# nihalsid/retrieval-fuse

Measured on AMD Instinct MI355X. Metric: 64^3 TSDF chunks/sec (retrieve+attend+refine), higher is better.
Workload: dtype f32

## Files before the change

### retrieval-fuse_amd/csrc/attention_fused.hip

```cpp
#include "common.h"
#include "attn_row.h"
#include "split_operand.h"
#include "philox.h"


typedef __attribute__((address_space(1))) const void* rf_gptr;
typedef __attribute__((address_space(3))) void* rf_lptr;

#define AM_HID 128
#define AM_OUT 32
#define AM_WAVES 16
#define AM_BUF_FLOATS (AM_HID * AM_HID)

static __host__ __device__ inline size_t am_layer_off(int n_in, int layer) {
    size_t o = 0;
    if (layer > 0) o += (size_t)n_in * AM_HID;
    if (layer > 1) o += (size_t)AM_HID * AM_HID;
    if (layer > 2) o += (size_t)AM_HID * AM_HID;
    if (layer > 3) o += (size_t)AM_HID * AM_OUT;
    return o;
}
static __host__ __device__ inline size_t am_bias_off(int n_in, int layer) { return am_layer_off(n_in, 4) + (size_t)layer * AM_HID; }

extern "C" size_t rf_attn_mlp_packed_floats(int n_in) { return am_bias_off(n_in, 3) + AM_OUT; }

struct AmPackArgs {
    const float* w[4];
    const float* b[4];
    float* img;
    int n_in;
};

__global__ void k_attn_mlp_pack(AmPackArgs a) {
    const size_t total = am_bias_off(a.n_in, 3) + AM_OUT;
    for (size_t i = (size_t)blockIdx.x * blockDim.x + threadIdx.x; i < total; i += (size_t)gridDim.x * blockDim.x) {
        float v;
        if (i >= am_layer_off(a.n_in, 4)) {
            const size_t bi = i - am_layer_off(a.n_in, 4);
            const int layer = (int)(bi / AM_HID) > 3 ? 3 : (int)(bi / AM_HID);
            v = a.b[layer][bi - (size_t)layer * AM_HID];
        } else {
            int layer = 0;
            while (layer < 3 && i >= am_layer_off(a.n_in, layer + 1)) ++layer;
            const size_t li = i - am_layer_off(a.n_in, layer);
            const int nin = layer == 0 ? a.n_in : AM_HID;
            const int ibn = layer == 3 ? AM_OUT / 16 : AM_HID / 16;
            const int r = (int)(li & 3), lane = (int)((li >> 2) & 63);
            const int ib = (int)((li >> 8) % ibn), kb = (int)((li >> 8) / ibn);
            v = a.w[layer][(size_t)(ib * 16 + (lane & 15)) * nin + kb * 16 + 4 * (lane >> 4) + r];
        }
        a.img[i] = v;
    }
}

extern "C" int rf_attn_mlp_pack(const float* w1, const float* b1, const float* w2, const float* b2, const float* w3, const float* b3,
                                const float* w4, const float* b4, int n_in, float* packed, void* stream) {
    RF_REQUIRE(w1 && b1 && w2 && b2 && w3 && b3 && w4 && b4 && packed, RF_E_INVALID, "rf_attn_mlp_pack: null pointer");
    RF_REQUIRE(n_in >= 16 && n_in <= AM_HID && n_in % 16 == 0, RF_E_UNSUPPORTED, "rf_attn_mlp_pack: n_in %d must be a multiple of 16 in 16..128", n_in);
    AmPackArgs a;
    a.w[0] = w1; a.w[1] = w2; a.w[2] = w3; a.w[3] = w4;
    a.b[0] = b1; a.b[1] = b2; a.b[2] = b3; a.b[3] = b4;
    a.img = packed; a.n_in = n_in;
    return rf_launch<k_attn_mlp_pack>("rf_attn_mlp_pack", dim3(256), dim3(256), (hipStream_t)stream, a);
}

struct AmArgs {
    const float* src;
    const float* img;
    const float* img2;
    float* out;
    int mode;
    int nrows, n_in, ntiles;
    int kv, c, s, t;
};

template <int IB>
__device__ __forceinline__ void am_layer(const float* wbuf, int kbn, const f32x4 (&hin)[8], f32x4 (&acc)[8], int lane) {
    constexpr int GRP = 2;
    constexpr int NG = IB / GRP;
    const float4* wv = reinterpret_cast<const float4*>(wbuf) + lane;
#pragma unroll
    for (int ib = 0; ib < IB; ++ib) acc[ib] = (f32x4){0.f, 0.f, 0.f, 0.f};
    float4 aw[2][GRP];
#pragma unroll
    for (int i = 0; i < GRP; ++i) aw[0][i] = wv[i * 64];
#pragma unroll
    for (int kb = 0; kb < 8; ++kb) {
        if (kb < kbn) {
#pragma unroll
            for (int gi = 0; gi < NG; ++gi) {
                const int st = kb * NG + gi, cur = st & 1, nxt = cur ^ 1;
                if (st + 1 < 8 * NG) {
#pragma unroll
                    for (int i = 0; i < GRP; ++i) aw[nxt][i] = wv[((st + 1) * GRP + i) * 64];
                }
#pragma unroll
                for (int i = 0; i < GRP; ++i) acc[gi * GRP + i] = __builtin_amdgcn_mfma_f32_16x16x4f32(aw[cur][i].x, hin[kb][0], acc[gi * GRP + i], 0, 0, 0);
#pragma unroll
                for (int i = 0; i < GRP; ++i) acc[gi * GRP + i] = __builtin_amdgcn_mfma_f32_16x16x4f32(aw[cur][i].y, hin[kb][1], acc[gi * GRP + i], 0, 0, 0);
#pragma unroll
                for (int i = 0; i < GRP; ++i) acc[gi * GRP + i] = __builtin_amdgcn_mfma_f32_16x16x4f32(aw[cur][i].z, hin[kb][2], acc[gi * GRP + i], 0, 0, 0);
#pragma unroll
                for (int i = 0; i < GRP; ++i) acc[gi * GRP + i] = __builtin_amdgcn_mfma_f32_16x16x4f32(aw[cur][i].w, hin[kb][3], acc[gi * GRP + i], 0, 0, 0);
            }
        }
    }
}

__global__ __launch_bounds__(AM_WAVES * 64) void k_attn_mlp(AmArgs a) {
    extern __shared__ __attribute__((aligned(16))) float smem[];
    const int tid = threadIdx.x, lane = tid & 63;
    const int wave = __builtin_amdgcn_readfirstlane(tid >> 6);
    const int g = lane >> 4, j = lane & 15;
    const int kb0 = a.n_in >> 4;

    auto dma_layer = [&](int layer) {
        const int npiece = layer == 0 ? kb0 * 8 : (layer == 3 ? (AM_HID / 16) * (AM_OUT / 16) : 64);
        const float* src = a.img + am_layer_off(a.n_in, layer);
        float* dst = smem + (layer & 1) * AM_BUF_FLOATS;
        for (int q = wave; q < npiece; q += AM_WAVES)
            __builtin_amdgcn_global_load_lds((rf_gptr)(src + q * 256 + lane * 4), (rf_lptr)(dst + q * 256), 16, 0, 0);
    };
    const float4* bias4 = reinterpret_cast<const float4*>(a.img + am_layer_off(a.n_in, 4));

    dma_layer(0);
    const int nwt = (a.ntiles + AM_WAVES - 1) / AM_WAVES;
    for (int wt = blockIdx.x; wt < nwt; wt += gridDim.x) {
        const int rt = wt * AM_WAVES + wave;
        const bool live = rt < a.ntiles;
        int row = rt * 16 + j;
        if (row >= a.nrows) row = a.nrows - 1;
        if (row < 0) row = 0;
        size_t orow = (size_t)row;
        f32x4 hin[8];
        if (a.mode == 0) {
            const float* p = a.src + (size_t)row * a.n_in + 4 * g;
#pragma unroll
            for (int kb = 0; kb < 8; ++kb) {
                if (kb < kb0) {
                    const float4 v = *reinterpret_cast<const float4*>(p + kb * 16);
                    hin[kb] = (f32x4){v.x, v.y, v.z, v.w};
                } else {
                    hin[kb] = (f32x4){0.f, 0.f, 0.f, 0.f};
                }
            }
        } else {
            const int r = a.s >> 1, t = a.t, q = a.s / t;
            const int r3 = r * r * r;
            const int vol = row / r3, prow = row - vol * r3;
            const int p2 = prow % r, p1 = (prow / r) % r, p0 = prow / (r * r);
            const int bb = vol / a.kv, k = vol - bb * a.kv;
            orow = ((size_t)bb * r3 + prow) * a.kv + k;
            const int d0 = 2 * p0 + (g & 1), d1 = 2 * p1, d2 = 2 * p2;
            const size_t t3 = (size_t)t * t * t;
            const size_t patch = (((size_t)vol * q + d0 / t) * q + d1 / t) * q + d2 / t;
            const float* p = a.src + (patch * a.c + (g >> 1)) * t3 + ((size_t)(d0 % t) * t + (d1 % t)) * t + (d2 % t);
#pragma unroll
            for (int kb = 0; kb < 8; ++kb) {
                if (kb < kb0) {
                    const float2 lo = *reinterpret_cast<const float2*>(p + (size_t)(2 * kb) * t3);
                    const float2 hi = *reinterpret_cast<const float2*>(p + (size_t)(2 * kb) * t3 + t);
                    hin[kb] = (f32x4){lo.x, lo.y, hi.x, hi.y};
                } else {
                    hin[kb] = (f32x4){0.f, 0.f, 0.f, 0.f};
                }
            }
        }

        f32x4 acc[8];
#pragma unroll
        for (int layer = 0; layer < 4; ++layer) {
            __syncthreads();
            if (layer < 3) dma_layer(layer + 1);
            else if (wt + (int)gridDim.x < nwt) dma_layer(0);
            const float* wbuf = smem + (layer & 1) * AM_BUF_FLOATS;
            if (layer < 3) {
                am_layer<8>(wbuf, layer == 0 ? kb0 : 8, hin, acc, lane);
#pragma unroll
                for (int ib = 0; ib < 8; ++ib) {
                    const float4 bz = bias4[layer * 32 + ib * 4 + g];
                    f32x4 v = acc[ib];
                    v[0] += bz.x; v[1] += bz.y; v[2] += bz.z; v[3] += bz.w;
#pragma unroll
                    for (int e = 0; e < 4; ++e) v[e] = v[e] > 0.f ? v[e] : v[e] * 0.01f;
                    hin[ib] = v;
                }
            } else {
                am_layer<2>(wbuf, 8, hin, acc, lane);
                if (live && rt * 16 + j < a.nrows) {
#pragma unroll
                    for (int ib = 0; ib < 2; ++ib) {
                        const float4 bz = bias4[3 * 32 + ib * 4 + g];
                        const float4 o = make_float4(acc[ib][0] + bz.x, acc[ib][1] + bz.y, acc[ib][2] + bz.z, acc[ib][3] + bz.w);
                        *reinterpret_cast<float4*>(a.out + orow * AM_OUT + ib * 16 + 4 * g) = o;
                    }
                }
            }
        }
    }
}


static __host__ __device__ inline int ams_steps(int n_in, int layer) { return layer == 0 ? (n_in / 16 + 1) / 2 : 4; }
static __host__ __device__ inline int ams_ibn(int layer) { return layer == 3 ? AM_OUT / 16 : AM_HID / 16; }
static __host__ __device__ inline size_t ams_layer_off(int n_in, int layer) {
    size_t o = 0;
    for (int l = 0; l < layer; ++l) o += (size_t)ams_steps(n_in, l) * ams_ibn(l) * 2 * 256;
    return o;
}
extern "C" size_t rf_attn_mlp_split_packed_floats(int n_in) { return ams_layer_off(n_in, 4); }

struct AmsPackArgs {
    const float* w[4];
    float* img;
    int n_in;
};

__global__ void k_attn_mlp_split_pack(AmsPackArgs a) {
    const size_t total = ams_layer_off(a.n_in, 4) / 4;
    for (size_t i = (size_t)blockIdx.x * blockDim.x + threadIdx.x; i < total; i += (size_t)gridDim.x * blockDim.x) {
        int layer = 0;
        while (layer < 3 && i * 4 >= ams_layer_off(a.n_in, layer + 1)) ++layer;
        const size_t li = i - ams_layer_off(a.n_in, layer) / 4;
        const int nin = layer == 0 ? a.n_in : AM_HID, ibn = ams_ibn(layer);
        const int lane = (int)(li & 63), piece = (int)((li >> 6) & 1);
        const int ib = (int)((li >> 7) % ibn), t = (int)((li >> 7) / ibn);
        const int feat = ib * 16 + (lane & 15), g = lane >> 4;
        h8 out;
#pragma unroll
        for (int j = 0; j < 8; ++j) {
            const int k = 16 * (2 * t + (j >> 2)) + 4 * g + (j & 3);
            _Float16 h, l;
            rf_split_weight(k < nin ? (double)a.w[layer][(size_t)feat * nin + k] : 0.0, h, l);
            out[j] = piece == 0 ? h : l;
        }
        reinterpret_cast<h8*>(a.img)[i] = out;
    }
}

extern "C" int rf_attn_mlp_split_pack(const float* w1, const float* w2, const float* w3, const float* w4, int n_in, float* packed, void* stream) {
    RF_REQUIRE(w1 && w2 && w3 && w4 && packed, RF_E_INVALID, "rf_attn_mlp_split_pack: null pointer");
    RF_REQUIRE(n_in >= 16 && n_in <= AM_HID && n_in % 16 == 0, RF_E_UNSUPPORTED, "rf_attn_mlp_split_pack: n_in %d must be a multiple of 16 in 16..128", n_in);
    AmsPackArgs a;
    a.w[0] = w1; a.w[1] = w2; a.w[2] = w3; a.w[3] = w4; a.img = packed; a.n_in = n_in;
    return rf_launch<k_attn_mlp_split_pack>("rf_attn_mlp_split_pack", dim3(256), dim3(256), (hipStream_t)stream, a);
}

typedef float am_f2 __attribute__((ext_vector_type(2)));
__device__ __forceinline__ void ams_split4(const f32x4& v, h8& h, h8& l, int o) {
#pragma unroll
    for (int e = 0; e < 4; e += 2) {
        const am_f2 s2 = (am_f2){v[e], v[e + 1]} * (am_f2){SPLIT_ACT_SCALE, SPLIT_ACT_SCALE};
        am_f2 x;
        x.x = rf_clamp_f16(s2.x);
        x.y = rf_clamp_f16(s2.y);
        const am_f2 xl = x * (am_f2){SPLIT_LO, SPLIT_LO};
        const _Float16 ha = (_Float16)x.x, hb = (_Float16)x.y;
        h[o + e] = ha; h[o + e + 1] = hb;
        l[o + e] = (_Float16)fmaf(-SPLIT_LO, (float)ha, xl.x);
        l[o + e + 1] = (_Float16)fmaf(-SPLIT_LO, (float)hb, xl.y);
    }
}

template <int IB>
__device__ __forceinline__ void ams_layer(const float* wbuf, int tn, const h8 (&bh)[4], const h8 (&bl)[4], f32x4 (&hi)[8], f32x4 (&lo)[8], int lane) {
    const h8* wv = reinterpret_cast<const h8*>(wbuf) + lane;
#pragma unroll
    for (int ib = 0; ib < IB; ++ib) { hi[ib] = (f32x4){0.f, 0.f, 0.f, 0.f}; lo[ib] = (f32x4){0.f, 0.f, 0.f, 0.f}; }
    h8 wh[2], wl[2];
    wh[0] = wv[0]; wl[0] = wv[64];
#pragma unroll
    for (int t = 0; t < 4; ++t) {
        if (t < tn) {
#pragma unroll
            for (int ib = 0; ib < IB; ++ib) {
                const int st = t * IB + ib, cur = st & 1, nxt = cur ^ 1;
                if (st + 1 < 4 * IB) { wh[nxt] = wv[(st + 1) * 128]; wl[nxt] = wv[(st + 1) * 128 + 64]; }
                hi[ib] = __builtin_amdgcn_mfma_f32_16x16x32_f16(wh[cur], bh[t], hi[ib], 0, 0, 0);
                lo[ib] = __builtin_amdgcn_mfma_f32_16x16x32_f16(wh[cur], bl[t], lo[ib], 0, 0, 0);
                lo[ib] = __builtin_amdgcn_mfma_f32_16x16x32_f16(wl[cur], bh[t], lo[ib], 0, 0, 0);
            }
        }
    }
}

#define AMS_WAVES 12
__global__ __launch_bounds__(AMS_WAVES * 64) void k_attn_mlp_split(AmArgs a) {
    extern __shared__ __attribute__((aligned(16))) float smem[];
    const int tid = threadIdx.x, lane = tid & 63;
    const int wave = __builtin_amdgcn_readfirstlane(tid >> 6);
    const int g = lane >> 4, j = lane & 15;
    const int kb0 = a.n_in >> 4, t0n = (kb0 + 1) >> 1;

    auto dma_layer = [&](int layer) {
        const int npiece = ams_steps(a.n_in, layer) * ams_ibn(layer) * 2;
        const float* src = a.img2 + ams_layer_off(a.n_in, layer);
        float* dst = smem + (layer & 1) * AM_BUF_FLOATS;
        for (int q = wave; q < npiece; q += AMS_WAVES)
            __builtin_amdgcn_global_load_lds((rf_gptr)(src + q * 256 + lane * 4), (rf_lptr)(dst + q * 256), 16, 0, 0);
    };
    const float4* bias4 = reinterpret_cast<const float4*>(a.img + am_layer_off(a.n_in, 4));

    dma_layer(0);
    const int nwt = (a.ntiles + AMS_WAVES - 1) / AMS_WAVES;
    for (int wt = blockIdx.x; wt < nwt; wt += gridDim.x) {
        const int rt = wt * AMS_WAVES + wave;
        const bool live = rt < a.ntiles;
        int row = rt * 16 + j;
        if (row >= a.nrows) row = a.nrows - 1;
        if (row < 0) row = 0;
        size_t orow = (size_t)row;
        h8 bh[4], bl[4];
#pragma unroll
        for (int t = 0; t < 4; ++t) { bh[t] = (h8){0, 0, 0, 0, 0, 0, 0, 0}; bl[t] = bh[t]; }
        if (a.mode == 0) {
            const float* p = a.src + (size_t)row * a.n_in + 4 * g;
#pragma unroll
            for (int kb = 0; kb < 8; ++kb) {
                if (kb < kb0) {
                    const float4 v = *reinterpret_cast<const float4*>(p + kb * 16);
                    ams_split4((f32x4){v.x, v.y, v.z, v.w}, bh[kb >> 1], bl[kb >> 1], 4 * (kb & 1));
                }
            }
        } else {
            const int r = a.s >> 1, t = a.t, q = a.s / t;
            const int r3 = r * r * r;
            const int vol = row / r3, prow = row - vol * r3;
            const int p2 = prow % r, p1 = (prow / r) % r, p0 = prow / (r * r);
            const int bb = vol / a.kv, k = vol - bb * a.kv;
            orow = ((size_t)bb * r3 + prow) * a.kv + k;
            const int d0 = 2 * p0 + (g & 1), d1 = 2 * p1, d2 = 2 * p2;
            const size_t t3 = (size_t)t * t * t;
            const size_t patch = (((size_t)vol * q + d0 / t) * q + d1 / t) * q + d2 / t;
            const float* p = a.src + (patch * a.c + (g >> 1)) * t3 + ((size_t)(d0 % t) * t + (d1 % t)) * t + (d2 % t);
#pragma unroll
            for (int kb = 0; kb < 8; ++kb) {
                if (kb < kb0) {
                    const float2 lo2 = *reinterpret_cast<const float2*>(p + (size_t)(2 * kb) * t3);
                    const float2 hi2 = *reinterpret_cast<const float2*>(p + (size_t)(2 * kb) * t3 + t);
                    ams_split4((f32x4){lo2.x, lo2.y, hi2.x, hi2.y}, bh[kb >> 1], bl[kb >> 1], 4 * (kb & 1));
                }
            }
        }

        f32x4 hi[8], lo[8];
#pragma unroll
        for (int layer = 0; layer < 4; ++layer) {
            __syncthreads();
            if (layer < 3) dma_layer(layer + 1);
            else if (wt + (int)gridDim.x < nwt) dma_layer(0);
            const float* wbuf = smem + (layer & 1) * AM_BUF_FLOATS;
            if (layer < 3) {
                ams_layer<8>(wbuf, layer == 0 ? t0n : 4, bh, bl, hi, lo, lane);
#pragma unroll
                for (int ib = 0; ib < 8; ++ib) {
                    const float4 bz = bias4[layer * 32 + ib * 4 + g];
                    const am_f2 c2 = {1.0f / SPLIT_LO, 1.0f / SPLIT_LO}, s2 = {0.01f, 0.01f};
                    const am_f2 va = __builtin_elementwise_fma((am_f2){lo[ib][0], lo[ib][1]}, c2, (am_f2){hi[ib][0], hi[ib][1]}) + (am_f2){bz.x, bz.y};
                    const am_f2 vb = __builtin_elementwise_fma((am_f2){lo[ib][2], lo[ib][3]}, c2, (am_f2){hi[ib][2], hi[ib][3]}) + (am_f2){bz.z, bz.w};
                    const am_f2 na = va * s2, nb = vb * s2;
                    const f32x4 v = {rf_max(va.x, na.x), rf_max(va.y, na.y), rf_max(vb.x, nb.x), rf_max(vb.y, nb.y)};
                    ams_split4(v, bh[ib >> 1], bl[ib >> 1], 4 * (ib & 1));
                }
            } else {
                ams_layer<2>(wbuf, 4, bh, bl, hi, lo, lane);
                if (live && rt * 16 + j < a.nrows) {
#pragma unroll
                    for (int ib = 0; ib < 2; ++ib) {
                        const float4 bz = bias4[3 * 32 + ib * 4 + g];
                        const float4 o = make_float4(rf_split_join(hi[ib][0], lo[ib][0]) + bz.x, rf_split_join(hi[ib][1], lo[ib][1]) + bz.y,
                                                     rf_split_join(hi[ib][2], lo[ib][2]) + bz.z, rf_split_join(hi[ib][3], lo[ib][3]) + bz.w);
                        *reinterpret_cast<float4*>(a.out + orow * AM_OUT + ib * 16 + 4 * g) = o;
                    }
                }
            }
        }
    }
}

static int am_launch(const AmArgs& a, hipStream_t st) {
    constexpr size_t lds = 2 * AM_BUF_FLOATS * sizeof(float);
    if (a.img2) return rf_launch<k_attn_mlp_split>("rf_attn_mlp", dim3(rf_blocks(a.ntiles, AMS_WAVES, 256)), dim3(AMS_WAVES * 64), lds, lds, st, a);
    return rf_launch<k_attn_mlp>("rf_attn_mlp", dim3(rf_blocks(a.ntiles, AM_WAVES, 256)), dim3(AM_WAVES * 64), lds, lds, st, a);
}

static int am_rows(const float* x, int rows, int n_in, const float* packed, const float* packed_split, float* out, void* stream);
extern "C" int rf_attn_mlp_rows(const float* x, int rows, int n_in, const float* packed, float* out, void* stream) {
    return am_rows(x, rows, n_in, packed, nullptr, out, stream);
}
extern "C" int rf_attn_mlp_split_rows(const float* x, int rows, int n_in, const float* packed, const float* packed_split, float* out, void* stream) {
    RF_REQUIRE(packed_split, RF_E_INVALID, "rf_attn_mlp_split_rows: null split image");
    return am_rows(x, rows, n_in, packed, packed_split, out, stream);
}
static int am_rows(const float* x, int rows, int n_in, const float* packed, const float* packed_split, float* out, void* stream) {
    RF_REQUIRE(x && packed && out && rows > 0, RF_E_INVALID, "rf_attn_mlp_rows: bad arguments");
    RF_REQUIRE(n_in >= 16 && n_in <= AM_HID && n_in % 16 == 0, RF_E_UNSUPPORTED, "rf_attn_mlp_rows: n_in %d must be a multiple of 16 in 16..128", n_in);
    AmArgs a;
    a.src = x; a.img = packed; a.img2 = packed_split; a.out = out; a.mode = 0; a.nrows = rows; a.n_in = n_in; a.ntiles = (rows + 15) / 16;
    a.kv = 1; a.c = 0; a.s = 0; a.t = 0;
    return am_launch(a, (hipStream_t)stream);
}

static int am_volume(const float* src, int b, int kv, int c, int s, int t, const float* packed, const float* packed_split, float* out, void* stream);
extern "C" int rf_attn_mlp_volume(const float* src, int b, int kv, int c, int s, int t, const float* packed, float* out, void* stream) {
    return am_volume(src, b, kv, c, s, t, packed, nullptr, out, stream);
}
extern "C" int rf_attn_mlp_split_volume(const float* src, int b, int kv, int c, int s, int t, const float* packed, const float* packed_split, float* out, void* stream) {
    RF_REQUIRE(packed_split, RF_E_INVALID, "rf_attn_mlp_split_volume: null split image");
    return am_volume(src, b, kv, c, s, t, packed, packed_split, out, stream);
}
static int am_volume(const float* src, int b, int kv, int c, int s, int t, const float* packed, const float* packed_split, float* out, void* stream) {
    RF_REQUIRE(src && packed && out && b > 0 && kv > 0 && c > 0 && s > 0 && t > 0, RF_E_INVALID, "rf_attn_mlp_volume: bad arguments");
    RF_REQUIRE(s % 2 == 0 && t % 2 == 0 && s % t == 0, RF_E_INVALID, "rf_attn_mlp_volume: edges s=%d t=%d must be even and t | s", s, t);
    RF_REQUIRE(c % 2 == 0 && c * 8 <= AM_HID, RF_E_UNSUPPORTED, "rf_attn_mlp_volume: %d channels (need an even count <= 16)", c);
    const long long rows = (long long)b * kv * (s / 2) * (s / 2) * (s / 2);
    RF_REQUIRE(rows < (1ll << 31) - 16, RF_E_UNSUPPORTED, "rf_attn_mlp_volume: too many rows");
    AmArgs a;
    a.src = src; a.img = packed; a.img2 = packed_split; a.out = out; a.mode = 1; a.nrows = (int)rows; a.n_in = c * 8; a.ntiles = (int)((rows + 15) / 16);
    a.kv = kv; a.c = c; a.s = s; a.t = t;
    return am_launch(a, (hipStream_t)stream);
}

__device__ __forceinline__ void rf_gumbel_row(unsigned long long seed, unsigned long long offset, int row, int K, float (&g)[RF_MAX_K]) {
#pragma unroll
    for (int q = 0; q < RF_MAX_K / 4; ++q) {
        if (4 * q < K) {
            unsigned c[4] = {(unsigned)row, (unsigned)q, (unsigned)offset, (unsigned)(offset >> 32)};
            rf_philox4x32_10(c, (unsigned)seed, (unsigned)(seed >> 32));
#pragma unroll
            for (int j = 0; j < 4; ++j) {
                const float u = ((float)(c[j] >> 8) + 0.5f) * (1.0f / 16777216.0f);
                g[4 * q + j] = -logf(-logf(u));
            }
        }
    }
}

__global__ __launch_bounds__(256) void k_attn_weights(const float* __restrict__ xf, const float* __restrict__ pf, const float* __restrict__ noise,
                                                      unsigned long long* __restrict__ rng, int rows, int K, int f, int mode, float sharpness,
                                                      float* __restrict__ w_out, float* __restrict__ sw_out, float* __restrict__ scores_out,
                                                      float* __restrict__ noise_out) {
    const unsigned long long seed = rng ? rng[0] : 0ull, offset = rng ? rng[1] : 0ull;
    for (int row = blockIdx.x * blockDim.x + threadIdx.x; row < rows; row += gridDim.x * blockDim.x) {
        float sc[RF_MAX_K], w[RF_MAX_K], sw, g[RF_MAX_K];
        const float* nrow = noise ? noise + (size_t)row * K : nullptr;
        if (!noise && mode == RF_ATTN_GUMBEL_HARD) {
            rf_gumbel_row(seed, offset, row, K, g);
            nrow = g;
        }
        rf_attn_row_weights(xf + (size_t)row * f, pf + (size_t)row * K * f, nrow, K, f, mode, sharpness, sc, w, sw);
#pragma unroll
        for (int k = 0; k < RF_MAX_K; ++k) {
            if (k < K) {
                w_out[(size_t)row * K + k] = w[k];
                if (scores_out) scores_out[(size_t)row * K + k] = sc[k];
                if (noise_out && nrow) noise_out[(size_t)row * K + k] = nrow[k];
            }
        }
        sw_out[row] = sw;
    }
    if (rng && !noise && mode == RF_ATTN_GUMBEL_HARD) {
        __syncthreads();
        if (threadIdx.x == 0) {
            __threadfence();
            if (atomicAdd(rng + 2, 1ull) == (unsigned long long)gridDim.x - 1ull) { rng[1] = offset + 1ull; rng[2] = 0ull; }
        }
    }
}

static int attn_weights_launch(const float* xf, const float* pf, const float* noise, unsigned long long* rng, int rows, int k, int f, int mode,
                               float sharpness, float* weights, float* switches, float* scores_out, float* noise_out, void* stream, const char* who) {
    RF_REQUIRE(xf && pf && weights && switches && rows > 0, RF_E_INVALID, "%s: bad arguments", who);
    RF_REQUIRE(k >= 1 && k <= RF_MAX_K, RF_E_UNSUPPORTED, "%s: K=%d outside 1..%d", who, k, RF_MAX_K);
    RF_REQUIRE(f >= 1 && f <= 128, RF_E_UNSUPPORTED, "%s: feature width %d outside 1..128", who, f);
    return rf_launch<k_attn_weights>(who, dim3(rf_blocks(rows, 256, 8192)), dim3(256), (hipStream_t)stream, xf, pf, noise, rng, rows, k, f, mode, sharpness, weights,
                                     switches, scores_out, noise_out);
}

extern "C" int rf_attn_weights(const float* xf, const float* pf, const float* noise, int rows, int k, int f, int mode, float sharpness,
                               float* weights, float* switches, float* scores_out, void* stream) {
    RF_REQUIRE(mode == RF_ATTN_SOFTMAX || (mode == RF_ATTN_GUMBEL_HARD && noise), RF_E_INVALID,
               "rf_attn_weights: Gumbel-hard mode needs the noise tensor (or rf_attn_weights_sampled)");
    return attn_weights_launch(xf, pf, noise, nullptr, rows, k, f, mode, sharpness, weights, switches, scores_out, nullptr, stream, "rf_attn_weights");
}

extern "C" int rf_attn_weights_sampled(const float* xf, const float* pf, int rows, int k, int f, float sharpness, void* rng_state,
                                       float* weights, float* switches, float* scores_out, float* noise_out, void* stream) {
    RF_REQUIRE(rng_state, RF_E_INVALID, "rf_attn_weights_sampled: null generator state");
    return attn_weights_launch(xf, pf, nullptr, reinterpret_cast<unsigned long long*>(rng_state), rows, k, f, RF_ATTN_GUMBEL_HARD, sharpness, weights,
                               switches, scores_out, noise_out, stream, "rf_attn_weights_sampled");
}

__global__ __launch_bounds__(256) void k_attn_blend(const float* __restrict__ x, const float* __restrict__ src, const float* __restrict__ w,
                                                    const float* __restrict__ sw, int b, int K, int c, int s, int t, float* __restrict__ out) {
    const int r = s >> 1, q = s / t;
    const size_t t3 = (size_t)t * t * t, total = (size_t)b * c * s * s * r;
    for (size_t i = (size_t)blockIdx.x * blockDim.x + threadIdx.x; i < total; i += (size_t)gridDim.x * blockDim.x) {
        const int p2 = (int)(i % r), d1 = (int)((i / r) % s), d0 = (int)((i / ((size_t)r * s)) % s);
        const int cc = (int)((i / ((size_t)r * s * s)) % c);
        const size_t bb = i / ((size_t)r * s * s * c);
        const size_t row = ((bb * r + (d0 >> 1)) * r + (d1 >> 1)) * r + p2;
        const int d2 = 2 * p2;
        const float swv = sw[row];
        float ws0 = 0.f, ws1 = 0.f;
        for (int k = 0; k < K; ++k) {
            const size_t vol = bb * K + k;
            const size_t patch = ((vol * q + d0 / t) * q + d1 / t) * q + d2 / t;
            const float2 pv = *reinterpret_cast<const float2*>(src + (patch * c + cc) * t3 + ((size_t)(d0 % t) * t + (d1 % t)) * t + (d2 % t));
            const float wk = w[row * K + k];
            ws0 = fmaf(wk, pv.x, ws0);
            ws1 = fmaf(wk, pv.y, ws1);
        }
        const float2 xv = reinterpret_cast<const float2*>(x)[i];
        reinterpret_cast<float2*>(out)[i] = make_float2(__fadd_rn(__fmul_rn(xv.x, 1.f - swv), __fmul_rn(ws0, swv)),
                                                        __fadd_rn(__fmul_rn(xv.y, 1.f - swv), __fmul_rn(ws1, swv)));
    }
}

extern "C" int rf_attn_blend(const float* x, const float* retrieved, int b, int k, int c, int s, int t, const float* weights,
                             const float* switches, float* out, void* stream) {
    RF_REQUIRE(x && retrieved && weights && switches && out && b > 0 && k > 0 && c > 0, RF_E_INVALID, "rf_attn_blend: bad arguments");
    RF_REQUIRE(s > 0 && t > 0 && s % 2 == 0 && t % 2 == 0 && s % t == 0, RF_E_INVALID, "rf_attn_blend: edges s=%d t=%d must be even and t | s", s, t);
    const size_t total = (size_t)b * c * s * s * (s / 2);
    return rf_launch<k_attn_blend>("rf_attn_blend", dim3(rf_blocks(total, 256, 16384)), dim3(256), (hipStream_t)stream, x, retrieved, weights, switches, b, k, c, s, t,
                                   out);
}
```

Baseline: 5189.

## Restructure attention blend kernel into plane-tiled blocks with vectorized loads and zero-weight skipping

```diff
diff --git a/retrieval-fuse_amd/csrc/attention_fused.hip b/retrieval-fuse_amd/csrc/attention_fused.hip
--- a/retrieval-fuse_amd/csrc/attention_fused.hip
+++ b/retrieval-fuse_amd/csrc/attention_fused.hip
@@ -491,37 +491,126 @@
                                switches, scores_out, noise_out, stream, "rf_attn_weights_sampled");
 }
 
-__global__ __launch_bounds__(256) void k_attn_blend(const float* __restrict__ x, const float* __restrict__ src, const float* __restrict__ w,
-                                                    const float* __restrict__ sw, int b, int K, int c, int s, int t, float* __restrict__ out) {
-    const int r = s >> 1, q = s / t;
-    const size_t t3 = (size_t)t * t * t, total = (size_t)b * c * s * s * r;
-    for (size_t i = (size_t)blockIdx.x * blockDim.x + threadIdx.x; i < total; i += (size_t)gridDim.x * blockDim.x) {
-        const int p2 = (int)(i % r), d1 = (int)((i / r) % s), d0 = (int)((i / ((size_t)r * s)) % s);
-        const int cc = (int)((i / ((size_t)r * s * s)) % c);
-        const size_t bb = i / ((size_t)r * s * s * c);
-        const size_t row = ((bb * r + (d0 >> 1)) * r + (d1 >> 1)) * r + p2;
-        const int d2 = 2 * p2;
-        const float swv = sw[row];
-        float ws0 = 0.f, ws1 = 0.f;
-        for (int k = 0; k < K; ++k) {
-            const size_t vol = bb * K + k;
-            const size_t patch = ((vol * q + d0 / t) * q + d1 / t) * q + d2 / t;
-            const float2 pv = *reinterpret_cast<const float2*>(src + (patch * c + cc) * t3 + ((size_t)(d0 % t) * t + (d1 % t)) * t + (d2 % t));
-            const float wk = w[row * K + k];
-            ws0 = fmaf(wk, pv.x, ws0);
-            ws1 = fmaf(wk, pv.y, ws1);
-        }
-        const float2 xv = reinterpret_cast<const float2*>(x)[i];
-        reinterpret_cast<float2*>(out)[i] = make_float2(__fadd_rn(__fmul_rn(xv.x, 1.f - swv), __fmul_rn(ws0, swv)),
-                                                        __fadd_rn(__fmul_rn(xv.y, 1.f - swv), __fmul_rn(ws1, swv)));
-    }
-}
+struct AbArgs {
+    const float* x;
+    const float* src;
+    const float* w;
+    const float* sw;
+    float* out;
+    int b, K, c, s, t;
+    int xw, rp;
+};
+
+template <int NP, bool WVEC>
+__global__ __launch_bounds__(256) void k_attn_blend(AbArgs a) {
+    const int s = a.s, t = a.t, r = s >> 1, q = s / t, K = a.K, c = a.c;
+    const int xl = (int)threadIdx.x % a.xw, rl = (int)threadIdx.x / a.xw;
+    if (rl >= a.rp) return;
+    const unsigned t3 = (unsigned)t * t * t, pstride = (unsigned)c * t3;
+    const size_t vstride = (size_t)c * s * s * s;
+    unsigned sx[NP];
+#pragma unroll
+    for (int j = 0; j < NP; ++j) {
+        const unsigned d2 = 2u * (unsigned)(NP * xl + j);
+        sx[j] = (d2 / t) * pstride + d2 % t;
+    }
+    const unsigned chunks = (unsigned)(s / a.rp), ngroups = (unsigned)a.b * c * s * chunks;
+    for (unsigned g = blockIdx.x; g < ngroups; g += gridDim.x) {
+        const unsigned ch = g % chunks, pl = g / chunks;
+        const unsigned d0 = pl % s, bc = pl / s;
+        const unsigned cc = bc % c, bb = bc / c;
+        const unsigned pz = d0 / t, zin = d0 - pz * t;
+        const size_t xbase = ((size_t)bc * s + d0) * s * s;
+        const size_t rowb = ((size_t)bb * r + (d0 >> 1)) * r * r;
+        const float* sbase = a.src + (size_t)bb * K * vstride + (size_t)pz * q * q * pstride + cc * t3 + zin * t * t;
+        const unsigned d1 = ch * a.rp + rl;
+        const unsigned py = d1 / t, yin = d1 - py * t;
+        const unsigned rlo = (d1 >> 1) * r + NP * xl;
+        const unsigned xo = d1 * s + 2 * NP * xl;
+        const float* sp = sbase + (py * q * pstride + yin * t);
+        const float* wr = a.w + (rowb + rlo) * K;
+
+        float xv[2 * NP], swv[NP];
+        if constexpr (NP == 2) {
+            const float4 v = *reinterpret_cast<const float4*>(a.x + xbase + xo);
+            xv[0] = v.x; xv[1] = v.y; xv[2] = v.z; xv[3] = v.w;
+            const float2 sv = *reinterpret_cast<const float2*>(a.sw + rowb + rlo);
+            swv[0] = sv.x; swv[NP - 1] = sv.y;
+        } else {
+            const float2 v = *reinterpret_cast<const float2*>(a.x + xbase + xo);
+            xv[0] = v.x; xv[1] = v.y;
+            swv[0] = a.sw[rowb + rlo];
+        }
+        float acc[NP][2];
+#pragma unroll
+        for (int j = 0; j < NP; ++j) acc[j][0] = acc[j][1] = 0.f;
+        for (int k0 = 0; k0 < K; k0 += 4) {
+            float wk[NP][4];
+#pragma unroll
+            for (int j = 0; j < NP; ++j) {
+                if constexpr (WVEC) {
+                    const float4 v = *reinterpret_cast<const float4*>(wr + (size_t)j * K + k0);
+                    wk[j][0] = v.x; wk[j][1] = v.y; wk[j][2] = v.z; wk[j][3] = v.w;
+                } else {
+#pragma unroll
+                    for (int i = 0; i < 4; ++i) wk[j][i] = k0 + i < K ? wr[(size_t)j * K + k0 + i] : 0.f;
+                }
+            }
+            float2 pv[4][NP];
+#pragma unroll
+            for (int i = 0; i < 4; ++i) {
+#pragma unroll
+                for (int j = 0; j < NP; ++j) {
+                    pv[i][j] = make_float2(0.f, 0.f);
+                    if (wk[j][i] != 0.f) pv[i][j] = *reinterpret_cast<const float2*>(sp + (size_t)(k0 + i) * vstride + sx[j]);
+                }
+            }
+#pragma unroll
+            for (int i = 0; i < 4; ++i) {
+#pragma unroll
+                for (int j = 0; j < NP; ++j) {
+                    if (wk[j][i] != 0.f) {
+                        acc[j][0] = fmaf(wk[j][i], pv[i][j].x, acc[j][0]);
+                        acc[j][1] = fmaf(wk[j][i], pv[i][j].y, acc[j][1]);
+                    }
+                }
+            }
+        }
+        float o[2 * NP];
+#pragma unroll
+        for (int j = 0; j < NP; ++j) {
+            o[2 * j] = __fadd_rn(__fmul_rn(xv[2 * j], 1.f - swv[j]), __fmul_rn(acc[j][0], swv[j]));
+            o[2 * j + 1] = __fadd_rn(__fmul_rn(xv[2 * j + 1], 1.f - swv[j]), __fmul_rn(acc[j][1], swv[j]));
+        }
+        if constexpr (NP == 2) *reinterpret_cast<float4*>(a.out + xbase + xo) = make_float4(o[0], o[1], o[2 * NP - 2], o[2 * NP - 1]);
+        else *reinterpret_cast<float2*>(a.out + xbase + xo) = make_float2(o[0], o[1]);
+    }
+}
+
+static inline bool rf_aligned(const void* p, size_t n) { return (reinterpret_cast<size_t>(p) & (n - 1)) == 0; }
 
 extern "C" int rf_attn_blend(const float* x, const float* retrieved, int b, int k, int c, int s, int t, const float* weights,
                              const float* switches, float* out, void* stream) {
     RF_REQUIRE(x && retrieved && weights && switches && out && b > 0 && k > 0 && c > 0, RF_E_INVALID, "rf_attn_blend: bad arguments");
     RF_REQUIRE(s > 0 && t > 0 && s % 2 == 0 && t % 2 == 0 && s % t == 0, RF_E_INVALID, "rf_attn_blend: edges s=%d t=%d must be even and t | s", s, t);
-    const size_t total = (size_t)b * c * s * s * (s / 2);
-    return rf_launch<k_attn_blend>("rf_attn_blend", dim3(rf_blocks(total, 256, 16384)), dim3(256), (hipStream_t)stream, x, retrieved, weights, switches, b, k, c, s, t,
-                                   out);
-}
+    RF_REQUIRE((size_t)c * s * s * s < (1ull << 31), RF_E_UNSUPPORTED, "rf_attn_blend: a volume of %d channels at edge %d is too large", c, s);
+    AbArgs a;
+    a.x = x; a.src = retrieved; a.w = weights; a.sw = switches; a.out = out;
+    a.b = b; a.K = k; a.c = c; a.s = s; a.t = t;
+    const int np = s % 4 == 0 && rf_aligned(x, 16) && rf_aligned(out, 16) && rf_aligned(switches, 8) ? 2 : 1;
+    a.xw = s / 2 / np;
+    RF_REQUIRE(a.xw <= 256, RF_E_UNSUPPORTED, "rf_attn_blend: edge %d is too large", s);
+    a.rp = 1;
+    for (int d = s; d > 1; --d)
+        if (s % d == 0 && d * a.xw <= 256) { a.rp = d; break; }
+    const bool wvec = k % 4 == 0 && rf_aligned(weights, 16);
+    const size_t groups = (size_t)b * c * s * (s / a.rp);
+    RF_REQUIRE(groups < (1ull << 31), RF_E_UNSUPPORTED, "rf_attn_blend: too many planes");
+    const dim3 grid(rf_blocks(groups, 1, 2048)), block(rf_round_up(a.rp * a.xw, 64));
+    if (np == 2) {
+        if (wvec) return rf_launch<k_attn_blend<2, true>>("rf_attn_blend", grid, block, (hipStream_t)stream, a);
+        return rf_launch<k_attn_blend<2, false>>("rf_attn_blend", grid, block, (hipStream_t)stream, a);
+    }
+    if (wvec) return rf_launch<k_attn_blend<1, true>>("rf_attn_blend", grid, block, (hipStream_t)stream, a);
+    return rf_launch<k_attn_blend<1, false>>("rf_attn_blend", grid, block, (hipStream_t)stream, a);
+}
```

Result: no change. 5208, median of 2 (+0.4%).
